# BrunoudA/MH-PPO

Hardware: AMD Instinct MI355X
Metric: env-steps/sec at 65536 envs × 4 agents, 1/2/4/8 MI355X + %HBM roofline (higher is better)
Workload: dtype f64 env / f32 nets; 1 GPU; config 3: 4cars nb_car=4 nb_ped=1 nb_lines=2, 65536 envs/GPU x 80 steps, full PPO iteration (rollout + returns + 10+10 epochs); envs_per_gpu=65536, agents=4, T=80, parallelism=dp1

## Files before the change

### include/mhppo.h

```cpp
#ifndef MHPPO_H
#define MHPPO_H
#include <stdint.h>

#ifdef __cplusplus
extern "C" {
#endif

#define MHPPO_OK 0
#define MHPPO_EINVAL -1
#define MHPPO_EHIP -2
#define MHPPO_ENOMEM -3
#define MHPPO_ENAN -4

#define MHPPO_COOP 0
#define MHPPO_4CARS 1
#define MHPPO_SCALABLE 2
#define MHPPO_NAIF 3
#define MHPPO_4CARS2 4
#define MHPPO_STOP 5
#define MHPPO_FIX_SCALABLE_LANES 1
#define MHPPO_GENERIC_STEP 2

typedef struct mhppo_env_cfg {
    int32_t variant;
// ... 111 lines not shown

int mhppo_libm_eval(int fn, uint64_t first, int64_t n, float *out, void *stream);

int mhppo_returns_scan(const double *rew, float *ret, int64_t B, int32_t T, double gamma, void *stream);
int mhppo_returns_scan_tm(const double *rew, float *ret, int64_t B, int32_t T, double gamma, void *stream);

typedef struct {
  float *obs, *act, *logp, *ret;
  double *rew;
} mhppo_bucket_dst;
int mhppo_bucket_scatter(const int64_t *pos, const int8_t *bucket, int64_t NS, int32_t T, const float *obs_tm,
                         const float *act_tm, const float *logp_tm, const float *ret_tm, const double *rew_tm,
                         const mhppo_bucket_dst *dst, void *stream);

int mhppo_bucket_scatter_sums(const int64_t *pos, const int8_t *bucket, int64_t NS, int32_t T, const float *obs_tm,
                              const float *act_tm, const float *logp_tm, const float *ret_tm, const double *rew_tm,
                              const mhppo_bucket_dst *dst, double *rew_sums, void *work, void *stream);

typedef struct {
  int64_t n_cross, n_wait, n_all, status;
  double counts[2];
  double rew_sums[3];
} mhppo_bucket_info;
int64_t mhppo_bucket_work_bytes(int64_t NS, int32_t T);
int mhppo_bucket_plan(int64_t N, int32_t S, int32_t P, int32_t dc, const int32_t *a_d, const int32_t *closest,
                      const uint8_t *exist, const int32_t *rec_of, const double *ep_min, const float *feat_d,
                      const float *logp_d, int32_t fix_bucket, const int32_t *status, int64_t *pos, int8_t *bucket,
                      float *c_obs, int32_t *c_act, float *c_logp, float *c_ret, mhppo_bucket_info *info,
                      void *work, void *stream);

int mhppo_adv_stats(const float *ret, const float *value, int64_t M, double *stats, void *stream);
int mhppo_adv_normalize(const float *ret, const float *value, int64_t M, const double *stats,
                        double m_global, float *adv, void *stream);

int mhppo_ppo_cont_fwd_bwd(const float *mu, const float *act, const float *logp_old,
                           const float *adv, int64_t M, double inv_m, float *dmu,
                           double *loss, void *stream);

int mhppo_ppo_choice_fwd_bwd(const float *probs, const float *logp_old, const float *adv,
                             int64_t M, const double *counts, double inv_m2, float *dprobs,
                             double *loss, void *stream);

#define MHPPO_TRAIN_EXACT_F32 0x100
int mhppo_mlp_train(int kind, int n_in, const float *packed, const float *X, int64_t M, const float *ret,
                    float *value, const float *act, const float *logp_old, const double *stats,
                    const double *counts, double m_global, float out_mean, float out_std, float *grad,
                    double *sums, void *stream);

int mhppo_mlp_train_pair(const float *packed_actor, const float *packed_critic, const float *X, int64_t M,
                         const float *ret, float *value, const float *act, const float *logp_old,
                         const double *stats, double m_global, float out_mean, float out_std,
                         float *grad_actor, double *sums_actor, float *grad_critic, double *sums_critic,
                         void *stream);

int mhppo_mse_fwd_bwd(const float *value, const float *ret, int64_t M, double inv_m, float *dv,
                      double *loss, void *stream);


int mhppo_mlp_forward(const mhppo_mlp *net, const float *X, int64_t M, float *out, void *stream);

#define MHPPO_DIAG_DSUM   0
#define MHPPO_DIAG_K3     1
#define MHPPO_DIAG_CLIP   2
#define MHPPO_DIAG_RATIO  3
#define MHPPO_DIAG_ENT    4
#define MHPPO_DIAG_E      5
#define MHPPO_DIAG_E2     6
#define MHPPO_DIAG_G      7
#define MHPPO_DIAG_G2     8
#define MHPPO_DIAG_V      9
#define MHPPO_DIAG_N     10
int64_t mhppo_ppo_diag_work_bytes(int64_t M);
int mhppo_ppo_diag(const mhppo_mlp *actor, const mhppo_mlp *critic, const float *X, int64_t M,
                   const void *act, const float *logp_old, const float *ret, double *sums,
                   void *work, void *stream);


int mhppo_gae_tm(const mhppo_mlp *critic0, const mhppo_mlp *critic1, const float *obs_tm,
                 const double *rew_tm, const int64_t *pos, const int8_t *bucket, int64_t B, int32_t T,
                 double gamma, double lambda, float *ret_tm, float *value_tm, void *stream);


#define MHPPO_EVS_ROWS       0
#define MHPPO_EVS_V0         1
#define MHPPO_EVS_V0_SQ      2
#define MHPPO_EVS_ABSA0      3
#define MHPPO_EVS_A0         4
#define MHPPO_EVS_A0_SQ      5
#define MHPPO_EVS_ABSVP0     6
#define MHPPO_EVS_ABSVP0_SQ  7
#define MHPPO_EVS_EPISODES   8
#define MHPPO_EVS_N_PED      9
#define MHPPO_EVS_PEDT      10
#define MHPPO_EVS_PEDT_SQ   11
#define MHPPO_EVS_WAIT      12
#define MHPPO_EVS_WAIT_SQ   13
#define MHPPO_EVS_N_CAR     14
#define MHPPO_EVS_CART      15
#define MHPPO_EVS_CART_SQ   16
#define MHPPO_EVS_FC        17
#define MHPPO_EVS_IC        18
#define MHPPO_EVS_N_YSPEED  19
#define MHPPO_EVS_YSPEED    20
#define MHPPO_EVS_YSPEED_SQ 21
#define MHPPO_EVS_N_YTIME   22
#define MHPPO_EVS_YTIME     23
// ... 72 lines not shown
```

### mh-ppo_amd/csrc/mlp_grad_reduce.h

```cpp
#pragma once
#include <hip/hip_runtime.h>

namespace {
constexpr int RG = 64;

template <class T>
__global__ void __launch_bounds__(256)
    k_grad_stage1(const T *gpart, const double *dpart, int nw, int np, double *tmp) {
  const int k = blockIdx.x * 256 + threadIdx.x;
  const int g = blockIdx.y, nd = np + 3, z = blockIdx.z;
  gpart += (size_t)z * nw * np;
  dpart += (size_t)z * nw * 3;
  tmp += (size_t)z * RG * nd;
  const int i0 = (int)((int64_t)g * nw / RG), i1 = (int)((int64_t)(g + 1) * nw / RG);
  double s = 0.0;
  if (k < np) {
#pragma unroll 16
    for (int i = i0; i < i1; i++) s += (double)gpart[(size_t)i * np + k];
  } else if (k < nd) {
    for (int i = i0; i < i1; i++) s += dpart[(size_t)i * 3 + (k - np)];
  } else {
    return;
  }
  tmp[(size_t)g * nd + k] = s;
}

constexpr int RD_COLS = 64, RD_GROUPS = 16;
__global__ void __launch_bounds__(RD_COLS * RD_GROUPS)
    k_grad_reduce_blocks(const double *gpart, const double *dpart, int nb, int np, float *grad, double *out3,
                         float *grad1, double *out3_1) {
  __shared__ double red[RD_GROUPS][RD_COLS];
  const int c = blockIdx.x * RD_COLS + (threadIdx.x & (RD_COLS - 1)), g = threadIdx.x / RD_COLS;
  const int nd = np + 3;
  if (blockIdx.y) {
    gpart += (size_t)nb * np;
    dpart += (size_t)nb * 3;
    grad = grad1;
    out3 = out3_1;
  }
  const int i0 = g * nb / RD_GROUPS, i1 = (g + 1) * nb / RD_GROUPS;
  double s = 0.0;
  if (c < np) {
#pragma unroll 16
    for (int i = i0; i < i1; i++) s += gpart[(size_t)i * np + c];
  } else if (c < nd) {
    for (int i = i0; i < i1; i++) s += dpart[(size_t)i * 3 + (c - np)];
  }
  red[g][threadIdx.x & (RD_COLS - 1)] = s;
  __syncthreads();
  if (g != 0 || c >= nd) return;
  double t = 0.0;
#pragma unroll
  for (int q = 0; q < RD_GROUPS; q++) t += red[q][threadIdx.x];
  if (c < np)
    grad[c] = (float)t;
  else if (out3)
    out3[c - np] += t;
}

__global__ void __launch_bounds__(256)
    k_grad_stage2(const double *tmp, int np, float *grad, double *out3, float *grad1, double *out3_1) {
  const int k = blockIdx.x * 256 + threadIdx.x, nd = np + 3;
  if (k >= nd) return;
  if (blockIdx.z) {
    tmp += (size_t)RG * nd;
    grad = grad1;
    out3 = out3_1;
  }
  double s = 0.0;
#pragma unroll 8
  for (int g = 0; g < RG; g++) s += tmp[(size_t)g * nd + k];
  if (k < np)
    grad[k] = (float)s;
  else if (out3)
    out3[k - np] += s;
}
}
```

### mh-ppo_amd/csrc/mlp_train.hip

```cpp
#include <hip/hip_runtime.h>
#include <stdint.h>

#include <algorithm>

#include "../../include/mhppo.h"
#include "common.h"
#include "mlp_tile.h"
#include "mlp_train_f32.h"
#include "mlp_x3_prims.h"
#include "mlp_x3.h"
#include "mlp_grad_reduce.h"

namespace {
struct Work {
  float *g = nullptr;
  double *d = nullptr;
  double *t = nullptr;
  int nw = 0;
  double *g64() const {
    static_assert(x3::WAVES * sizeof(float) >= sizeof(double), "a block's wave slots hold its float64 partial");
    return reinterpret_cast<double *>(g);
  }
};
constexpr int WORK_STREAMS = 4;
Work g_work[mhppo::MAX_DEVICES][WORK_STREAMS];
hipStream_t g_work_stream[mhppo::MAX_DEVICES][WORK_STREAMS];
int g_work_used[mhppo::MAX_DEVICES] = {0};
bool ensure_work(Work &wk, int slots) {
  if (wk.nw >= slots) return true;
  if (wk.g) (void)hipFree(wk.g);
  if (wk.d) (void)hipFree(wk.d);
  if (wk.t) (void)hipFree(wk.t);
  if (hipMalloc(&wk.g, sizeof(float) * (size_t)slots * NW_MAX) != hipSuccess ||
      hipMalloc(&wk.d, sizeof(double) * (size_t)slots * 3) != hipSuccess ||
      hipMalloc(&wk.t, sizeof(double) * (size_t)2 * RG * (NW_MAX + 3)) != hipSuccess) {
    wk = Work{};
    return false;
  }
  wk.nw = slots;
  return true;
}
Work *device_work(int dev, hipStream_t s) {
  int k = 0;
  while (k < g_work_used[dev] && g_work_stream[dev][k] != s) k++;
  if (k == g_work_used[dev]) {
    if (k == WORK_STREAMS) return nullptr;
    g_work_stream[dev][k] = s;
    g_work_used[dev] = k + 1;
  }
  return &g_work[dev][k];
}

struct Launch {
  Work *wk;
  int blocks, nw;
};
enum XAlign { X_ANY, X_16B_BEFORE_LOOKUP, X_16B_AFTER_LOOKUP };
int prepare_launch(hipStream_t s, int64_t M, const float *X, XAlign xa, int waves, int nets, Launch &L) {
  if (M > ((int64_t)1 << 40)) return set_error(MHPPO_EINVAL, "M too large");
  const bool misaligned = ((uintptr_t)X & 15) != 0;
  if (xa == X_16B_BEFORE_LOOKUP && misaligned)
    return set_error(MHPPO_EINVAL, "X must be 16-byte aligned (LDS-DMA rows)");
  int dev = 0;
  CHECK_HIP(hipGetDevice(&dev));
  if (dev < 0 || dev >= mhppo::MAX_DEVICES) return set_error(MHPPO_EINVAL, "device %d >= %d", dev, mhppo::MAX_DEVICES);
  L.wk = device_work(dev, s);
  if (!L.wk) return set_error(MHPPO_EINVAL, "train passes on more than %d streams of one device", WORK_STREAMS);
  if (xa == X_16B_AFTER_LOOKUP && misaligned)
    return set_error(MHPPO_EINVAL, "X must be 16-byte aligned (LDS-DMA rows)");
  const int64_t tiles = (M + 31) / 32;
  L.blocks = (int)std::max<int64_t>(1, std::min<int64_t>(mhppo::device_cus(dev), (tiles + waves - 1) / waves));
  L.nw = L.blocks * waves;
  if (!ensure_work(*L.wk, nets * L.nw)) return set_error(MHPPO_ENOMEM, "mlp_train partials");
  return MHPPO_OK;
}

using X3Kernel = decltype(&k_mlp_train_x3<K_CRITIC, x3::G13S>);
struct X3Launch {
  X3Kernel kernel;
  int lds_bytes;
};
template <int KIND, class G>
constexpr X3Launch x3_of() { return {k_mlp_train_x3<KIND, G>, G::LDS_BYTES}; }
X3Launch x3_kernel(int kind, int n_in) {
  using namespace x3;
  const bool critic = kind == K_CRITIC;
  if (n_in == NIN_CONT && kind != K_CHOICE) return critic ? x3_of<K_CRITIC, G13S>() : x3_of<K_CONT, G13S>();
  if (n_in <= 15) return critic ? x3_of<K_CRITIC, GV16>() : x3_of<K_CHOICE, GC16>();
  if (n_in <= 31) return critic ? x3_of<K_CRITIC, GV32>() : x3_of<K_CHOICE, GC32>();
  if (n_in == 54) return critic ? x3_of<K_CRITIC, GV54>() : x3_of<K_CHOICE, GC54>();
  return critic ? x3_of<K_CRITIC, GV64>() : x3_of<K_CHOICE, GC64>();
}
using F32Launch = decltype(&launch<K_CRITIC, 7, true>);
F32Launch f32_launcher(int kind, int n_in) {
  if (n_in == NIN_CONT && kind != K_CHOICE)
    return kind == K_CRITIC ? launch<K_CRITIC, 7, true> : launch<K_CONT, 7, true>;
  static constexpr F32Launch CRITIC[6] = {launch<K_CRITIC, 8, false>,  launch<K_CRITIC, 12, false>,
                                          launch<K_CRITIC, 16, false>, launch<K_CRITIC, 24, false>,
                                          launch<K_CRITIC, 28, false>, launch<K_CRITIC, 32, false>};
  static constexpr F32Launch CHOICE[6] = {launch<K_CHOICE, 8, false>,  launch<K_CHOICE, 12, false>,
                                          launch<K_CHOICE, 16, false>, launch<K_CHOICE, 24, false>,
                                          launch<K_CHOICE, 28, false>, launch<K_CHOICE, 32, false>};
  const int w = n_in <= 16 ? 0 : (n_in <= 24 ? 1 : (n_in <= 32 ? 2 : (n_in <= 48 ? 3 : (n_in <= 56 ? 4 : 5))));
  return (kind == K_CRITIC ? CRITIC : CHOICE)[w];
}
}

#ifdef MHPPO_TIMING
extern "C" int mhppo_debug_timing_train(unsigned long long *out16) {
  CHECK_HIP(hipDeviceSynchronize());
  CHECK_HIP(hipMemcpyFromSymbol(out16, HIP_SYMBOL(g_timing), sizeof(unsigned long long) * 16));
  unsigned long long z[16] = {0};
  CHECK_HIP(hipMemcpyToSymbol(HIP_SYMBOL(g_timing), z, sizeof(z)));
  return MHPPO_OK;
}
#endif

extern "C" int mhppo_mlp_train(int kind, int n_in, const float *packed, const float *X, int64_t M, const float *ret,
                               float *value, const float *act, const float *logp_old, const double *stats,
                               const double *counts, double m_global, float out_mean, float out_std, float *grad,
                               double *sums, void *stream) {
  const bool exact = (kind & MHPPO_TRAIN_EXACT_F32) != 0;
  kind &= ~MHPPO_TRAIN_EXACT_F32;
  if (!grad || M < 0 || kind < K_CRITIC || kind > K_CHOICE || n_in < 1 || n_in > NIN_MAX)
    return set_error(MHPPO_EINVAL, "bad argument (kind 0..2 [| MHPPO_TRAIN_EXACT_F32], 1 <= n_in <= %d)", NIN_MAX);
  hipStream_t s = (hipStream_t)stream;
  const int np = n_params(n_in, kind == K_CHOICE ? 2 : 1);
  if (M == 0) {
    CHECK_HIP(hipMemsetAsync(grad, 0, sizeof(float) * np, s));
    return MHPPO_OK;
  }
  if (!packed || !X || !ret || !value) return set_error(MHPPO_EINVAL, "null packed/X/ret/value");
  if (kind == K_CONT && (n_in != NIN_CONT || !act || !logp_old || !stats))
    return set_error(MHPPO_EINVAL, "continuous actor pass needs n_in 13 and act/logp_old/stats");
  if (kind == K_CHOICE && (!logp_old || !stats || (!counts && !act)))
    return set_error(MHPPO_EINVAL, "choice actor pass needs logp_old/stats and counts (or act for per-row mode)");
  const bool pf = n_in == NIN_CONT && kind != K_CHOICE;
  const bool split = !exact && (pf || n_in <= x3::NIN_X3C);
  const int waves = split ? x3::WAVES : (pf ? 8 : 4);
  Launch L;
  const int rc = prepare_launch(s, M, X, pf ? X_16B_BEFORE_LOOKUP : (split ? X_16B_AFTER_LOOKUP : X_ANY), waves, 1, L);
  if (rc != MHPPO_OK) return rc;
  Work &wk = *L.wk;
  const dim3 grid((unsigned)L.blocks);
  if (split) {
    const X3Launch k = x3_kernel(kind, n_in);
    hipLaunchKernelGGL(k.kernel, grid, dim3(64 * x3::WAVES), k.lds_bytes, s, packed, X, n_in, M, ret, value, act,
                       logp_old, stats, counts, m_global, out_mean, out_std, wk.g64(), wk.d);
    hipLaunchKernelGGL(k_grad_reduce_blocks, dim3((np + 3 + RD_COLS - 1) / RD_COLS), dim3(RD_COLS * RD_GROUPS), 0, s,
                       wk.g64(), wk.d, L.blocks, np, grad, sums, nullptr, nullptr);
  } else {
    f32_launcher(kind, n_in)(grid, s, packed, X, n_in, M, ret, value, act, logp_old, stats, counts, m_global, out_mean,
                             out_std, wk.g, wk.d);
    hipLaunchKernelGGL(k_grad_stage1<float>, dim3((np + 3 + 255) / 256, RG), dim3(256), 0, s, wk.g, wk.d, L.nw, np,
                       wk.t);
    hipLaunchKernelGGL(k_grad_stage2, dim3((np + 3 + 255) / 256), dim3(256), 0, s, wk.t, np, grad, sums, nullptr,
                       nullptr);
  }
  CHECK_HIP(hipGetLastError());
  return MHPPO_OK;
}

extern "C" int mhppo_mlp_train_pair(const float *packed_actor, const float *packed_critic, const float *X, int64_t M,
                                    const float *ret, float *value, const float *act, const float *logp_old,
                                    const double *stats, double m_global, float out_mean, float out_std,
                                    float *grad_actor, double *sums_actor, float *grad_critic, double *sums_critic,
                                    void *stream) {
  if (!grad_actor || !grad_critic || M < 0) return set_error(MHPPO_EINVAL, "bad argument");
  hipStream_t s = (hipStream_t)stream;
  const int np = n_params(NIN_CONT, 1);
  if (M == 0) {
    CHECK_HIP(hipMemsetAsync(grad_actor, 0, sizeof(float) * np, s));
    CHECK_HIP(hipMemsetAsync(grad_critic, 0, sizeof(float) * np, s));
    return MHPPO_OK;
  }
  if (!packed_actor || !packed_critic || !X || !ret || !value || !act || !logp_old || !stats)
    return set_error(MHPPO_EINVAL, "null pointer");
  Launch L;
  const int rc = prepare_launch(s, M, X, X_16B_BEFORE_LOOKUP, x3::WAVES, 2, L);
  if (rc != MHPPO_OK) return rc;
  Work &wk = *L.wk;
  hipLaunchKernelGGL(k_mlp_train_x3_pair, dim3((unsigned)L.blocks), dim3(64 * x3::WAVES), x3::G13::LDS_BYTES_PAIR, s,
                     packed_actor, packed_critic, X, M, ret, value, act, logp_old, stats, m_global, out_mean, out_std,
                     wk.g64(), wk.d);
  hipLaunchKernelGGL(k_grad_reduce_blocks, dim3((np + 3 + RD_COLS - 1) / RD_COLS, 2), dim3(RD_COLS * RD_GROUPS), 0, s,
                     wk.g64(), wk.d, L.blocks, np, grad_actor, sums_actor, grad_critic, sums_critic);
  CHECK_HIP(hipGetLastError());
  return MHPPO_OK;
}
```

### mh-ppo_amd/mhppo/_lib.py

```python
import ctypes
import os

HERE = os.path.dirname(os.path.abspath(__file__))
LIB_PATH = os.environ.get("MHPPO_LIB") or os.path.join(HERE, "lib", "libmhppo.so")

P = ctypes.c_void_p
I32 = ctypes.c_int32
I64 = ctypes.c_int64
U64 = ctypes.c_uint64
F64 = ctypes.c_double


class EnvCfg(ctypes.Structure):
    _fields_ = [
        ("variant", I32), ("n_envs", I32), ("nb_car", I32), ("nb_ped", I32), ("nb_lines", I32),
        ("max_episode", I32), ("sin_model", I32), ("flags", I32), ("dt", F64),
        ("car_b", F64 * 4), ("ped_b", F64 * 8), ("cross_b", F64 * 2), ("seed_base", U64),
        ("env_id_offset", U64),
    ]


class Mlp(ctypes.Structure):
    _fields_ = [("packed", P), ("n_in", I32), ("n_out", I32), ("kind", I32), ("reserved", I32),
                ("mean", ctypes.c_float), ("std", ctypes.c_float)]


class BucketDst(ctypes.Structure):
    _fields_ = [("obs", P), ("act", P), ("logp", P), ("ret", P), ("rew", P)]


class RolloutBufs(ctypes.Structure):
    _fields_ = [("feat_d", P), ("probs_d", P), ("logp_d", P), ("a_d", P), ("closest", P),
                ("feat_c", P), ("out_c", P), ("obs", P), ("obs_c", P), ("act", P), ("logp", P),
                ("rew", P), ("ep_min", P), ("exist", P), ("rows", P), ("T", I32),
                ("flags", I32), ("status", P), ("parts", I32), ("reserved", I32), ("rec_of", P)]


class EvalBufs(ctypes.Structure):
    _fields_ = [("obs", P), ("a_d", P), ("trig", P), ("ep_min", P), ("obs_hist", P), ("acts", P), ("rews_c", P),
                ("rews_d", P), ("waiting", P), ("saved", P), ("T", I32), ("reserved", I32)]


class PolicyNoise(ctypes.Structure):
    _fields_ = [("tape", P), ("forced", P), ("key", U64), ("first_env", U64), ("t", I64)]


class AdamSeg(ctypes.Structure):
    _fields_ = [("param", P), ("grad", P), ("exp_avg", P), ("exp_avg_sq", P), ("step", P), ("n", I64)]


ADAM_MAX_NETS, ADAM_MAX_SEGS = 8, 8


class AdamNet(ctypes.Structure):
    _fields_ = [("seg", AdamSeg * ADAM_MAX_SEGS), ("n_seg", I32), ("reserved", I32), ("t", I64), ("alpha", F64),
                ("bias2", F64), ("beta1", F64), ("beta2", F64), ("eps", F64)]


_SIGS = {
    "mhppo_env_create": (I32, [ctypes.POINTER(EnvCfg), I32, ctypes.POINTER(P)]),
    "mhppo_env_destroy": (None, [P]),
    "mhppo_env_obs_dim": (I32, [P]),
    "mhppo_env_slots": (I32, [P]),
    "mhppo_env_reward_slots": (I32, [P]),
    "mhppo_env_state_dim": (I32, [P]),
    "mhppo_env_reset": (I32, [P, P, P]),
    "mhppo_env_choix_test": (I32, [P, P, P]),
    "mhppo_env_state_bytes": (I64, [P]),
    "mhppo_env_export": (I32, [P, P, P]),
    "mhppo_env_import": (I32, [P, P, P]),
    "mhppo_env_step": (I32, [P, P, P, P, P, P, P]),
    "mhppo_env_get_state": (I32, [P, P, P]),
    "mhppo_env_get_rng": (I32, [P, P, P, P]),
    "mhppo_env_events": (I32, [P, P, P]),
    "mhppo_choice_dim": (I32, [P]),
    "mhppo_rollout_begin": (I32, [P, ctypes.POINTER(Mlp), P, P, ctypes.POINTER(RolloutBufs), P]),
    "mhppo_rollout_step": (I32, [P, ctypes.POINTER(Mlp), ctypes.POINTER(Mlp), P, I32,
                                 ctypes.POINTER(RolloutBufs), P]),
    "mhppo_rollout_policy": (I32, [P, ctypes.POINTER(Mlp), ctypes.POINTER(Mlp), ctypes.POINTER(RolloutBufs), P]),
    "mhppo_rollout_sample_env": (I32, [P, P, I32, ctypes.POINTER(RolloutBufs), P]),
    "mhppo_rollout_policy_part": (I32, [P, ctypes.POINTER(Mlp), ctypes.POINTER(Mlp), ctypes.POINTER(RolloutBufs), I32,
                                        P]),
    "mhppo_rollout_sample_env_part": (I32, [P, P, I32, ctypes.POINTER(RolloutBufs), I32, P]),
    "mhppo_kernel_timing_begin": (I32, [I32]),
    "mhppo_kernel_timing_end": (I32, [ctypes.POINTER(ctypes.c_double), ctypes.POINTER(I32)]),
    "mhppo_kernel_timing_end_each": (I32, [P, I32, ctypes.POINTER(I32)]),
    "mhppo_eval_step": (I32, [P, ctypes.POINTER(Mlp), ctypes.POINTER(Mlp), ctypes.POINTER(Mlp), I32,
                              ctypes.POINTER(EvalBufs), P]),
    "mhppo_rollout_check": (I32, [ctypes.POINTER(RolloutBufs), P]),
    "mhppo_philox_normal": (I32, [U64, U64, P, I64, P]),
    "mhppo_philox_uniform": (I32, [U64, U64, P, I64, P]),
    "mhppo_philox_normal_2d": (I32, [U64, U64, U64, P, I64, I64, P]),
    "mhppo_libm_eval": (I32, [I32, U64, I64, P, P]),
    "mhppo_returns_scan": (I32, [P, P, I64, I32, F64, P]),
    "mhppo_returns_scan_tm": (I32, [P, P, I64, I32, F64, P]),
    "mhppo_bucket_scatter": (I32, [P, P, I64, I32] + [P] * 7),
    "mhppo_bucket_scatter_sums": (I32, [P, P, I64, I32] + [P] * 9),
    "mhppo_bucket_work_bytes": (I64, [I64, I32]),
    "mhppo_bucket_plan": (I32, [I64, I32, I32, I32] + [P] * 7 + [I32] + [P] * 10),
    "mhppo_adv_stats": (I32, [P, P, I64, P, P]),
    "mhppo_adv_normalize": (I32, [P, P, I64, P, F64, P, P]),
    "mhppo_ppo_cont_fwd_bwd": (I32, [P, P, P, P, I64, F64, P, P, P]),
    "mhppo_ppo_choice_fwd_bwd": (I32, [P, P, P, I64, P, F64, P, P, P]),
    "mhppo_mse_fwd_bwd": (I32, [P, P, I64, F64, P, P, P]),
    "mhppo_mlp_train": (I32, [I32, I32, P, P, I64, P, P, P, P, P, P, F64, ctypes.c_float, ctypes.c_float, P, P, P]),
    "mhppo_mlp_train_pair": (I32, [P, P, P, I64, P, P, P, P, P, F64, ctypes.c_float, ctypes.c_float, P, P, P, P, P]),
    "mhppo_mlp_forward": (I32, [ctypes.POINTER(Mlp), P, I64, P, P]),
    "mhppo_ppo_diag_work_bytes": (I64, [I64]),
    "mhppo_ppo_diag": (I32, [ctypes.POINTER(Mlp), ctypes.POINTER(Mlp), P, I64, P, P, P, P, P, P]),
    "mhppo_gae_tm": (I32, [ctypes.POINTER(Mlp), ctypes.POINTER(Mlp), P, P, P, P, I64, I32, F64, F64, P, P, P]),
    "mhppo_eval_stats_bytes": (I64, [P]),
    "mhppo_eval_stats_begin": (I32, [P, P, P]),
    "mhppo_eval_stats_row": (I32, [P, P, I32, I32, P, P]),
    "mhppo_eval_stats_fold": (I32, [P, P, P, P]),
    "mhppo_adam_clip": (I32, [P, I32, F64, P, P]),
    "mhppo_batch_shuffle": (I32, [I32, I64, P, P, P, P, U64, I32, P, P, P, P, P, P]),
    "mhppo_policy_dims": (I32, [ctypes.POINTER(EnvCfg), P]),
    "mhppo_policy_decide": (I32, [ctypes.POINTER(EnvCfg), ctypes.POINTER(Mlp), P, I64, P, P, P]),
    "mhppo_policy_act": (I32, [ctypes.POINTER(EnvCfg), ctypes.POINTER(Mlp), ctypes.POINTER(Mlp), P, P, I64, P, P]),
    "mhppo_policy_sample_decide": (I32, [ctypes.POINTER(EnvCfg), ctypes.POINTER(Mlp), P, I64,
                                         ctypes.POINTER(PolicyNoise)] + [P] * 8),
    "mhppo_policy_sample_act": (I32, [ctypes.POINTER(EnvCfg), ctypes.POINTER(Mlp), ctypes.POINTER(Mlp), P, P, P, I64,
                                      ctypes.POINTER(PolicyNoise)] + [P] * 6),
    "mhppo_last_error": (ctypes.c_char_p, []),
    "mhppo_version": (ctypes.c_char_p, []),
}

_lib = None


class MhppoError(RuntimeError):
    pass


class MhppoNaNError(MhppoError, ValueError):
    """MHPPO_ENAN: a NaN policy output was sampled (the reference raises ValueError there)."""

ENAN = -4
MHPPO_ROLLOUT_VALU_POLICY = 1
MHPPO_ROLLOUT_VALU_UNSORTED = 2


def lib():
    global _lib
    if _lib is None:
        if not os.path.exists(LIB_PATH):
            raise MhppoError(f"{LIB_PATH} is missing: build it with `python -c 'import __graft_entry__ as g; g.build()'`")
        L = ctypes.CDLL(LIB_PATH)
        for name, (res, args) in _SIGS.items():
            fn = getattr(L, name)
            fn.restype = res
            fn.argtypes = args
        _lib = L
    return _lib


def declared_symbols():
    return list(_SIGS)

# ... 52 lines not shown
```

### mh-ppo_amd/mhppo/ppo.py

```python
import contextlib
import ctypes
import math
import os

import torch
import torch.distributed as dist

from . import _lib
from .adam import adam_clip_steps, adam_clip_sumsq, adam_clip_torch, adam_steps, clip_forget, fold_1024_4


_FORCE_COLLECTIVES = False


def set_force_collectives(flag=True):
    global _FORCE_COLLECTIVES
    _FORCE_COLLECTIVES = bool(flag)


def _dp():
    if not (dist.is_available() and dist.is_initialized()):
        return False
    return _FORCE_COLLECTIVES or dist.get_world_size() > 1

# ... 273 lines not shown
        self.per_row = per_row
        self.exact = bool(exact)


PIPELINE_PAIRS = {"0": False, "1": True}.get(os.environ.get("MHPPO_PIPELINE_PAIRS", ""), None)
PAIR_MAX_ROWS = 2_000_000


def _use_pair(h):
    if h.kind != "c" or h.exact:
        return False
    return PIPELINE_PAIRS if PIPELINE_PAIRS is not None else h.m <= PAIR_MAX_ROWS


class _HeadPlan:

    def __init__(self, h):
        cont = h.kind == "c"
        self.akind = KIND_CONT if cont else KIND_CHOICE
        _check_net(KIND_CRITIC, h.critic)
        _check_net(self.akind, h.actor)
        self.obs, self.ret = _obs_rows(h.obs), h.ret.float().contiguous()
        self.M = self.obs.shape[0]
        self.lp = h.logp.float().contiguous()
        self.act = h.act.float().contiguous() if (cont or h.per_row) else None
        self.counts = None if (cont or h.per_row) else h.counts
        self.V = torch.empty(self.M, dtype=torch.float32, device=self.obs.device)
        self.n_in = h.actor.n_in
        self.keep = (h.actor.flat(), h.critic.flat())
        self.wa, self.wc = self.keep[0].data_ptr(), self.keep[1].data_ptr()
        self.ga, self.gc = h.actor.grad_flat().data_ptr(), h.critic.grad_flat().data_ptr()
        self.mean, self.std = float(h.actor.mean), float(h.actor.std)
        self.flags = TRAIN_EXACT_F32 if h.exact else 0
        self.pair = _use_pair(h) and self.M > 0
        self.x, self.r, self.v, self.l = (t.data_ptr() for t in (self.obs, self.ret, self.V, self.lp))
        self.a, self.cn = _addr(self.act), _addr(self.counts)


def _critic_pass(p, h, sums, st):
    _launch_train(KIND_CRITIC, p.flags, p.n_in, p.wc, p.x, p.M, p.r, p.v, None, None, None, None, h.m, 0.0, 1.0, p.gc,
                  sums.data_ptr(), st)


def _actor_pass(p, h, stats, sums, st):
    _launch_train(p.akind, p.flags, p.n_in, p.wa, p.x, p.M, p.r, p.v, p.a, p.l, stats.data_ptr(), p.cn, h.m, p.mean,
                  p.std, p.ga, sums.data_ptr(), st)


def _pair_pass(p, h, stats, sums_a, sums_c, st):
    _launch_pair(p.wa, p.wc, p.x, p.M, p.r, p.v, p.a, p.l, stats.data_ptr(), h.m, p.mean, p.std, p.ga,
                 sums_a.data_ptr(), p.gc, sums_c.data_ptr(), st)


def _on_device(dev):
    return torch.cuda.device(dev) if dev.type == "cuda" else contextlib.nullcontext()


def _reduce_and_step(nets, opts, bucket, max_grad_norm, norms_out):
    if bucket is not None:
        bucket.allreduce(nets)
    else:
        _allreduce_net_grads(*nets)
    if max_grad_norm is None:
        adam_steps(opts)
    elif opts:
        adam_steps(opts, max_grad_norm, norms_out)


def train_epoch(heads, bucket=None, max_grad_norm=None, norms_out=None):
    H = len(heads)
    dev = heads[0].obs.device
    with _on_device(dev):
        st = torch.cuda.current_stream(dev).cuda_stream if dev.type == "cuda" else None
        sums = torch.zeros(2 * H, 3, dtype=torch.float64, device=dev)
        plans = [_HeadPlan(h) for h in heads]
        for i, (p, h) in enumerate(zip(plans, heads)):
            _critic_pass(p, h, sums[i], st)
        stats = sums[:H, 1:3].reshape(-1).contiguous()
        _allreduce_(stats)
        for i, (p, h) in enumerate(zip(plans, heads)):
            _actor_pass(p, h, stats[2 * i:2 * i + 2], sums[H + i], st)
        _reduce_and_step([n for h in heads for n in (h.actor, h.critic)],
                         [o for h in heads for o in (h.opt_actor, h.opt_critic)], bucket, max_grad_norm, norms_out)
    return [(sums[H + i, 0:1], sums[i, 0:1]) for i in range(H)]


TRAIN_STREAMS = max(1, int(os.environ.get("MHPPO_TRAIN_STREAMS", "1")))
_SIDE_STREAMS = {}


def _side_streams(dev, n):
    if dev.type != "cuda" or n <= 0:
        return []
    key = (dev.index if dev.index is not None else torch.cuda.current_device(), n)
    if key not in _SIDE_STREAMS:
        _SIDE_STREAMS[key] = [torch.cuda.Stream(device=dev) for _ in range(n)]
    return _SIDE_STREAMS[key]


def train_epochs(heads, n_epochs, bucket=None, max_grad_norm=None):
    H = len(heads)
    dev = heads[0].obs.device
    with _on_device(dev):
        norms = None
        if max_grad_norm is not None:
            norms = torch.full((n_epochs, 2 * H), math.nan, dtype=torch.float64, device=dev)
        all_sums = torch.zeros(n_epochs + 1, 2 * H, 3, dtype=torch.float64, device=dev)
        dp = _dp()
        plans = [_HeadPlan(h) for h in heads]
        main = torch.cuda.current_stream(dev) if dev.type == "cuda" else None
        side = _side_streams(dev, min(TRAIN_STREAMS, H) - 1)
        streams = [main] + side
        handles = [None if s is None else s.cuda_stream for s in streams]
        same_stream = contextlib.nullcontext()
        stats = None
        out = [[None, None] for _ in range(H)]
        for k in range(n_epochs + 1):
            sums = all_sums[k]
            crit = k < n_epochs
            trained = []
            if side:
                fork = torch.cuda.Event()
                fork.record(main)
                for sd in side:
                    sd.wait_event(fork)
            for i, h in enumerate(heads):
                p = plans[i]
                sc, sa = sums[i], sums[H + i]
                j = i % len(streams)
                st = handles[j]
                with (torch.cuda.stream(streams[j]) if side else same_stream):
                    stp = None
                    if k > 0:
                        stp = stats[2 * i:2 * i + 2] if dp else all_sums[k - 1, i, 1:3]
                    if k > 0 and crit and p.pair:
                        _pair_pass(p, h, stp, sa, sc, st)
                    else:
                        if k > 0:
                            _actor_pass(p, h, stp, sa, st)
                        if crit:
                            _critic_pass(p, h, sc, st)
                if k > 0:
                    trained.append(h.actor)
                    out[i][0] = sums[H + i, 0:1]
                if crit:
                    trained.append(h.critic)
                    out[i][1] = sums[i, 0:1]
            for sd in side:
                main.wait_stream(sd)
            if crit and dp:
                stats = sums[:H, 1:3].reshape(-1).contiguous()
                _allreduce_(stats)
            opts = ([h.opt_actor for h in heads] if k > 0 else []) + ([h.opt_critic for h in heads] if crit else [])
            nout = None
            if norms is not None:
                off = (k - 1) * 2 * H + H if k > 0 else 0
                nout = norms.view(-1)[off:off + len(opts)]
            _reduce_and_step(trained, opts, bucket, max_grad_norm, nout)
    if norms is not None:
        return [tuple(o) for o in out], norms
    return [tuple(o) for o in out]



class _SliceHead:

    def __init__(self, h, m):
        self.actor, self.critic, self.kind, self.m = h.actor, h.critic, h.kind, float(m)


class _SlicePlan:

    def __init__(self, p, b0, b1, counts):
        for k in ("akind", "n_in", "wa", "wc", "ga", "gc", "mean", "std", "flags", "keep"):
            setattr(self, k, getattr(p, k))
        self.pair = False
        self.M = b1 - b0
        self.obs, self.ret, self.V, self.lp = p.obs[b0:b1], p.ret[b0:b1], p.V[b0:b1], p.lp[b0:b1]
        self.act = None if p.act is None else p.act[b0:b1]
        self.counts = counts
        self.x, self.r, self.v, self.l = p.x + 4 * self.n_in * b0, p.r + 4 * b0, p.v + 4 * b0, p.l + 4 * b0
        self.a = None if p.a is None else p.a + 4 * b0
        self.cn = _addr(counts)


def train_minibatches(heads, n_epochs, K, key_fn, bucket=None, max_grad_norm=None, slice_m=None):
    from . import shuffle
    H, K = len(heads), int(K)
    if K < 1:
        raise ValueError(f"K must be >= 1, not {K}")
    dev = heads[0].obs.device
    with _on_device(dev):
        st = torch.cuda.current_stream(dev).cuda_stream if dev.type == "cuda" else None
        dp = _dp()
        n_choice = sum(1 for h in heads if h.kind != "c" and not h.per_row)
        counts_all = torch.zeros(max(1, n_choice), K, 2, dtype=torch.float64, device=dev)
        srcs, dsts, cnts, plans = [], [], [], []
        for h in heads:
            fl = h.kind == "c" or h.per_row
            act = h.act.float().contiguous() if fl else h.act.to(torch.int32).contiguous()
            src = (h.obs.float().contiguous(), act, h.logp.float().contiguous(), h.ret.float().contiguous())
            dst = tuple(torch.empty_like(t) for t in src)
# ... 63 lines not shown
```

Baseline: 79.63 million env-steps/s.

## Batch all per-epoch train passes into one native call with shared gradient reduce

Adds mhppo_train_step, which takes a table of actor, critic and pair passes for every head. It launches them in one native call across at most two streams, joins the streams, and then runs a single table-driven gradient-reduce kernel over all nets. This replaces many per-head Python/ctypes calls, per-pass reduce launches and torch side-stream event plumbing. The goal is lower host dispatch and launch overhead in the PPO epochs, at the cost of a serialized reduce after the join and a limit of two streams.

```diff
diff --git a/include/mhppo.h b/include/mhppo.h
--- a/include/mhppo.h
+++ b/include/mhppo.h
@@ -187,6 +187,31 @@
                          const double *stats, double m_global, float out_mean, float out_std,
                          float *grad_actor, double *sums_actor, float *grad_critic, double *sums_critic,
                          void *stream);
+
+#define MHPPO_TRAIN_STEP_MAX_PASSES 16
+typedef struct mhppo_train_pass {
+  int32_t pair;
+  int32_t head;
+  int32_t kind;
+  int32_t n_in;
+  const float *packed;
+  const float *packed_critic;
+  const float *X;
+  int64_t M;
+  const float *ret;
+  float *value;
+  const float *act;
+  const float *logp_old;
+  const double *stats;
+  const double *counts;
+  double m_global;
+  float out_mean, out_std;
+  float *grad;
+  double *sums;
+  float *grad_critic;
+  double *sums_critic;
+} mhppo_train_pass;
+int mhppo_train_step(const mhppo_train_pass *passes, int n_passes, int streams, void *stream);
 
 int mhppo_mse_fwd_bwd(const float *value, const float *ret, int64_t M, double inv_m, float *dv,
                       double *loss, void *stream);
diff --git a/mh-ppo_amd/csrc/mlp_grad_reduce.h b/mh-ppo_amd/csrc/mlp_grad_reduce.h
--- a/mh-ppo_amd/csrc/mlp_grad_reduce.h
+++ b/mh-ppo_amd/csrc/mlp_grad_reduce.h
@@ -1,5 +1,7 @@
 #pragma once
 #include <hip/hip_runtime.h>
+
+#include "../../include/mhppo.h"
 
 namespace {
 constexpr int RG = 64;
@@ -26,18 +28,22 @@
 }
 
 constexpr int RD_COLS = 64, RD_GROUPS = 16;
-__global__ void __launch_bounds__(RD_COLS * RD_GROUPS)
-    k_grad_reduce_blocks(const double *gpart, const double *dpart, int nb, int np, float *grad, double *out3,
-                         float *grad1, double *out3_1) {
+struct ReduceNet {
+  const double *gpart, *dpart;
+  float *grad;
+  double *out3;
+  int nb, np;
+};
+constexpr int RD_MAX_NETS = 2 * MHPPO_TRAIN_STEP_MAX_PASSES;
+struct ReduceTable {
+  ReduceNet net[RD_MAX_NETS];
+};
+__global__ void __launch_bounds__(RD_COLS * RD_GROUPS) k_grad_reduce_blocks(const ReduceTable tab) {
   __shared__ double red[RD_GROUPS][RD_COLS];
   const int c = blockIdx.x * RD_COLS + (threadIdx.x & (RD_COLS - 1)), g = threadIdx.x / RD_COLS;
-  const int nd = np + 3;
-  if (blockIdx.y) {
-    gpart += (size_t)nb * np;
-    dpart += (size_t)nb * 3;
-    grad = grad1;
-    out3 = out3_1;
-  }
+  const ReduceNet &n = tab.net[blockIdx.y];
+  const double *gpart = n.gpart, *dpart = n.dpart;
+  const int nb = n.nb, np = n.np, nd = np + 3;
   const int i0 = g * nb / RD_GROUPS, i1 = (g + 1) * nb / RD_GROUPS;
   double s = 0.0;
   if (c < np) {
@@ -53,9 +59,15 @@
 #pragma unroll
   for (int q = 0; q < RD_GROUPS; q++) t += red[q][threadIdx.x];
   if (c < np)
-    grad[c] = (float)t;
-  else if (out3)
-    out3[c - np] += t;
+    n.grad[c] = (float)t;
+  else if (n.out3)
+    n.out3[c - np] += t;
+}
+inline void launch_reduce_blocks(const ReduceTable &tab, int nets, hipStream_t s) {
+  int np = 0;
+  for (int i = 0; i < nets; i++) np = tab.net[i].np > np ? tab.net[i].np : np;
+  hipLaunchKernelGGL(k_grad_reduce_blocks, dim3((np + 3 + RD_COLS - 1) / RD_COLS, nets), dim3(RD_COLS * RD_GROUPS), 0,
+                     s, tab);
 }
 
 __global__ void __launch_bounds__(256)
diff --git a/mh-ppo_amd/csrc/mlp_train.hip b/mh-ppo_amd/csrc/mlp_train.hip
--- a/mh-ppo_amd/csrc/mlp_train.hip
+++ b/mh-ppo_amd/csrc/mlp_train.hip
@@ -55,6 +55,10 @@
   Work *wk;
   int blocks, nw;
 };
+int grid_blocks(int dev, int64_t M, int waves) {
+  const int64_t tiles = (M + 31) / 32;
+  return (int)std::max<int64_t>(1, std::min<int64_t>(mhppo::device_cus(dev), (tiles + waves - 1) / waves));
+}
 enum XAlign { X_ANY, X_16B_BEFORE_LOOKUP, X_16B_AFTER_LOOKUP };
 int prepare_launch(hipStream_t s, int64_t M, const float *X, XAlign xa, int waves, int nets, Launch &L) {
   if (M > ((int64_t)1 << 40)) return set_error(MHPPO_EINVAL, "M too large");
@@ -68,8 +72,7 @@
   if (!L.wk) return set_error(MHPPO_EINVAL, "train passes on more than %d streams of one device", WORK_STREAMS);
   if (xa == X_16B_AFTER_LOOKUP && misaligned)
     return set_error(MHPPO_EINVAL, "X must be 16-byte aligned (LDS-DMA rows)");
-  const int64_t tiles = (M + 31) / 32;
-  L.blocks = (int)std::max<int64_t>(1, std::min<int64_t>(mhppo::device_cus(dev), (tiles + waves - 1) / waves));
+  L.blocks = grid_blocks(dev, M, waves);
   L.nw = L.blocks * waves;
   if (!ensure_work(*L.wk, nets * L.nw)) return set_error(MHPPO_ENOMEM, "mlp_train partials");
   return MHPPO_OK;
@@ -104,6 +107,84 @@
   const int w = n_in <= 16 ? 0 : (n_in <= 24 ? 1 : (n_in <= 32 ? 2 : (n_in <= 48 ? 3 : (n_in <= 56 ? 4 : 5))));
   return (kind == K_CRITIC ? CRITIC : CHOICE)[w];
 }
+
+int check_single(int kind, int n_in, const float *packed, const float *X, int64_t M, const float *ret,
+                 const float *value, const float *act, const float *logp_old, const double *stats,
+                 const double *counts, const float *grad) {
+  if (!grad || M < 0 || kind < K_CRITIC || kind > K_CHOICE || n_in < 1 || n_in > NIN_MAX)
+    return set_error(MHPPO_EINVAL, "bad argument (kind 0..2 [| MHPPO_TRAIN_EXACT_F32], 1 <= n_in <= %d)", NIN_MAX);
+  if (M == 0) return MHPPO_OK;
+  if (!packed || !X || !ret || !value) return set_error(MHPPO_EINVAL, "null packed/X/ret/value");
+  if (kind == K_CONT && (n_in != NIN_CONT || !act || !logp_old || !stats))
+    return set_error(MHPPO_EINVAL, "continuous actor pass needs n_in 13 and act/logp_old/stats");
+  if (kind == K_CHOICE && (!logp_old || !stats || (!counts && !act)))
+    return set_error(MHPPO_EINVAL, "choice actor pass needs logp_old/stats and counts (or act for per-row mode)");
+  return MHPPO_OK;
+}
+int check_pair(const float *packed_actor, const float *packed_critic, const float *X, int64_t M, const float *ret,
+               const float *value, const float *act, const float *logp_old, const double *stats,
+               const float *grad_actor, const float *grad_critic) {
+  if (!grad_actor || !grad_critic || M < 0) return set_error(MHPPO_EINVAL, "bad argument");
+  if (M == 0) return MHPPO_OK;
+  if (!packed_actor || !packed_critic || !X || !ret || !value || !act || !logp_old || !stats)
+    return set_error(MHPPO_EINVAL, "null pointer");
+  return MHPPO_OK;
+}
+struct SingleShape {
+  bool pf, split;
+  int waves, np;
+};
+SingleShape single_shape(int kind, int n_in, bool exact) {
+  SingleShape sh;
+  sh.pf = n_in == NIN_CONT && kind != K_CHOICE;
+  sh.split = !exact && (sh.pf || n_in <= x3::NIN_X3C);
+  sh.waves = sh.split ? x3::WAVES : (sh.pf ? 8 : 4);
+  sh.np = n_params(n_in, kind == K_CHOICE ? 2 : 1);
+  return sh;
+}
+
+struct Step {
+  hipStream_t side = nullptr;
+  hipEvent_t fork = nullptr, join = nullptr;
+  double *g = nullptr, *d = nullptr;
+  size_t ng = 0, nd = 0;
+};
+Step g_step[mhppo::MAX_DEVICES];
+int ensure_step_lane(Step &st) {
+  if (st.side) return MHPPO_OK;
+  hipStream_t side = nullptr;
+  hipEvent_t fork = nullptr, join = nullptr;
+  if (hipStreamCreateWithFlags(&side, hipStreamNonBlocking) != hipSuccess ||
+      hipEventCreateWithFlags(&fork, hipEventDisableTiming) != hipSuccess ||
+      hipEventCreateWithFlags(&join, hipEventDisableTiming) != hipSuccess) {
+    if (join) (void)hipEventDestroy(join);
+    if (fork) (void)hipEventDestroy(fork);
+    if (side) (void)hipStreamDestroy(side);
+    return set_error(MHPPO_EHIP, "mhppo_train_step: side stream / events");
+  }
+  st.side = side, st.fork = fork, st.join = join;
+  return MHPPO_OK;
+}
+bool ensure_step_work(Step &st, size_t ng, size_t nd) {
+  if (st.ng < ng) {
+    if (st.g) (void)hipFree(st.g);
+    st.g = nullptr, st.ng = 0;
+    if (hipMalloc(&st.g, sizeof(double) * ng) != hipSuccess) return false;
+    st.ng = ng;
+  }
+  if (st.nd < nd) {
+    if (st.d) (void)hipFree(st.d);
+    st.d = nullptr, st.nd = 0;
+    if (hipMalloc(&st.d, sizeof(double) * nd) != hipSuccess) return false;
+    st.nd = nd;
+  }
+  return true;
+}
+int check_rows(int64_t M, const float *X, bool need_16b) {
+  if (M > ((int64_t)1 << 40)) return set_error(MHPPO_EINVAL, "M too large");
+  if (need_16b && ((uintptr_t)X & 15) != 0) return set_error(MHPPO_EINVAL, "X must be 16-byte aligned (LDS-DMA rows)");
+  return MHPPO_OK;
+}
 }
 
 #ifdef MHPPO_TIMING
@@ -116,42 +197,53 @@
 }
 #endif
 
+namespace {
+void launch_x3(int kind, int n_in, int blocks, hipStream_t s, const float *packed, const float *X, int64_t M,
+               const float *ret, float *value, const float *act, const float *logp_old, const double *stats,
+               const double *counts, double m_global, float out_mean, float out_std, double *gpart, double *dpart) {
+  const X3Launch k = x3_kernel(kind, n_in);
+  hipLaunchKernelGGL(k.kernel, dim3((unsigned)blocks), dim3(64 * x3::WAVES), k.lds_bytes, s, packed, X, n_in, M, ret,
+                     value, act, logp_old, stats, counts, m_global, out_mean, out_std, gpart, dpart);
+}
+void launch_x3_pair(int blocks, hipStream_t s, const float *packed_actor, const float *packed_critic, const float *X,
+                    int64_t M, const float *ret, float *value, const float *act, const float *logp_old,
+                    const double *stats, double m_global, float out_mean, float out_std, double *gpart,
+                    double *dpart) {
+  hipLaunchKernelGGL(k_mlp_train_x3_pair, dim3((unsigned)blocks), dim3(64 * x3::WAVES), x3::G13::LDS_BYTES_PAIR, s,
+                     packed_actor, packed_critic, X, M, ret, value, act, logp_old, stats, m_global, out_mean, out_std,
+                     gpart, dpart);
+}
+}
+
 extern "C" int mhppo_mlp_train(int kind, int n_in, const float *packed, const float *X, int64_t M, const float *ret,
                                float *value, const float *act, const float *logp_old, const double *stats,
                                const double *counts, double m_global, float out_mean, float out_std, float *grad,
                                double *sums, void *stream) {
   const bool exact = (kind & MHPPO_TRAIN_EXACT_F32) != 0;
   kind &= ~MHPPO_TRAIN_EXACT_F32;
-  if (!grad || M < 0 || kind < K_CRITIC || kind > K_CHOICE || n_in < 1 || n_in > NIN_MAX)
-    return set_error(MHPPO_EINVAL, "bad argument (kind 0..2 [| MHPPO_TRAIN_EXACT_F32], 1 <= n_in <= %d)", NIN_MAX);
+  const int rc0 = check_single(kind, n_in, packed, X, M, ret, value, act, logp_old, stats, counts, grad);
+  if (rc0 != MHPPO_OK) return rc0;
   hipStream_t s = (hipStream_t)stream;
-  const int np = n_params(n_in, kind == K_CHOICE ? 2 : 1);
+  const SingleShape sh = single_shape(kind, n_in, exact);
+  const int np = sh.np;
   if (M == 0) {
     CHECK_HIP(hipMemsetAsync(grad, 0, sizeof(float) * np, s));
     return MHPPO_OK;
   }
-  if (!packed || !X || !ret || !value) return set_error(MHPPO_EINVAL, "null packed/X/ret/value");
-  if (kind == K_CONT && (n_in != NIN_CONT || !act || !logp_old || !stats))
-    return set_error(MHPPO_EINVAL, "continuous actor pass needs n_in 13 and act/logp_old/stats");
-  if (kind == K_CHOICE && (!logp_old || !stats || (!counts && !act)))
-    return set_error(MHPPO_EINVAL, "choice actor pass needs logp_old/stats and counts (or act for per-row mode)");
-  const bool pf = n_in == NIN_CONT && kind != K_CHOICE;
-  const bool split = !exact && (pf || n_in <= x3::NIN_X3C);
-  const int waves = split ? x3::WAVES : (pf ? 8 : 4);
   Launch L;
-  const int rc = prepare_launch(s, M, X, pf ? X_16B_BEFORE_LOOKUP : (split ? X_16B_AFTER_LOOKUP : X_ANY), waves, 1, L);
+  const int rc = prepare_launch(s, M, X, sh.pf ? X_16B_BEFORE_LOOKUP : (sh.split ? X_16B_AFTER_LOOKUP : X_ANY),
+                                sh.waves, 1, L);
   if (rc != MHPPO_OK) return rc;
   Work &wk = *L.wk;
-  const dim3 grid((unsigned)L.blocks);
-  if (split) {
-    const X3Launch k = x3_kernel(kind, n_in);
-    hipLaunchKernelGGL(k.kernel, grid, dim3(64 * x3::WAVES), k.lds_bytes, s, packed, X, n_in, M, ret, value, act,
-                       logp_old, stats, counts, m_global, out_mean, out_std, wk.g64(), wk.d);
-    hipLaunchKernelGGL(k_grad_reduce_blocks, dim3((np + 3 + RD_COLS - 1) / RD_COLS), dim3(RD_COLS * RD_GROUPS), 0, s,
-                       wk.g64(), wk.d, L.blocks, np, grad, sums, nullptr, nullptr);
+  if (sh.split) {
+    launch_x3(kind, n_in, L.blocks, s, packed, X, M, ret, value, act, logp_old, stats, counts, m_global, out_mean,
+              out_std, wk.g64(), wk.d);
+    ReduceTable tab = {};
+    tab.net[0] = {wk.g64(), wk.d, grad, sums, L.blocks, np};
+    launch_reduce_blocks(tab, 1, s);
   } else {
-    f32_launcher(kind, n_in)(grid, s, packed, X, n_in, M, ret, value, act, logp_old, stats, counts, m_global, out_mean,
-                             out_std, wk.g, wk.d);
+    f32_launcher(kind, n_in)(dim3((unsigned)L.blocks), s, packed, X, n_in, M, ret, value, act, logp_old, stats, counts,
+                             m_global, out_mean, out_std, wk.g, wk.d);
     hipLaunchKernelGGL(k_grad_stage1<float>, dim3((np + 3 + 255) / 256, RG), dim3(256), 0, s, wk.g, wk.d, L.nw, np,
                        wk.t);
     hipLaunchKernelGGL(k_grad_stage2, dim3((np + 3 + 255) / 256), dim3(256), 0, s, wk.t, np, grad, sums, nullptr,
@@ -166,7 +258,9 @@
                                     const double *stats, double m_global, float out_mean, float out_std,
                                     float *grad_actor, double *sums_actor, float *grad_critic, double *sums_critic,
                                     void *stream) {
-  if (!grad_actor || !grad_critic || M < 0) return set_error(MHPPO_EINVAL, "bad argument");
+  const int rc0 = check_pair(packed_actor, packed_critic, X, M, ret, value, act, logp_old, stats, grad_actor,
+                             grad_critic);
+  if (rc0 != MHPPO_OK) return rc0;
   hipStream_t s = (hipStream_t)stream;
   const int np = n_params(NIN_CONT, 1);
   if (M == 0) {
@@ -174,17 +268,109 @@
     CHECK_HIP(hipMemsetAsync(grad_critic, 0, sizeof(float) * np, s));
     return MHPPO_OK;
   }
-  if (!packed_actor || !packed_critic || !X || !ret || !value || !act || !logp_old || !stats)
-    return set_error(MHPPO_EINVAL, "null pointer");
   Launch L;
   const int rc = prepare_launch(s, M, X, X_16B_BEFORE_LOOKUP, x3::WAVES, 2, L);
   if (rc != MHPPO_OK) return rc;
   Work &wk = *L.wk;
-  hipLaunchKernelGGL(k_mlp_train_x3_pair, dim3((unsigned)L.blocks), dim3(64 * x3::WAVES), x3::G13::LDS_BYTES_PAIR, s,
-                     packed_actor, packed_critic, X, M, ret, value, act, logp_old, stats, m_global, out_mean, out_std,
-                     wk.g64(), wk.d);
-  hipLaunchKernelGGL(k_grad_reduce_blocks, dim3((np + 3 + RD_COLS - 1) / RD_COLS, 2), dim3(RD_COLS * RD_GROUPS), 0, s,
-                     wk.g64(), wk.d, L.blocks, np, grad_actor, sums_actor, grad_critic, sums_critic);
+  launch_x3_pair(L.blocks, s, packed_actor, packed_critic, X, M, ret, value, act, logp_old, stats, m_global, out_mean,
+                 out_std, wk.g64(), wk.d);
+  ReduceTable tab = {};
+  tab.net[0] = {wk.g64(), wk.d, grad_actor, sums_actor, L.blocks, np};
+  tab.net[1] = {wk.g64() + (size_t)L.blocks * np, wk.d + (size_t)L.blocks * 3, grad_critic, sums_critic, L.blocks, np};
+  launch_reduce_blocks(tab, 2, s);
   CHECK_HIP(hipGetLastError());
   return MHPPO_OK;
 }
+
+extern "C" int mhppo_train_step(const mhppo_train_pass *passes, int n_passes, int streams, void *stream) {
+  if (n_passes < 0 || n_passes > MHPPO_TRAIN_STEP_MAX_PASSES || (n_passes > 0 && !passes) || streams < 1 || streams > 2)
+    return set_error(MHPPO_EINVAL, "mhppo_train_step: 0 <= n_passes <= %d pass records, 1 or 2 streams",
+                     MHPPO_TRAIN_STEP_MAX_PASSES);
+  for (int i = 0; i < n_passes; i++) {
+    const mhppo_train_pass &p = passes[i];
+    if (p.head < 0) return set_error(MHPPO_EINVAL, "mhppo_train_step: pass %d has a negative head", i);
+    int rc;
+    bool need_16b = true;
+    if (p.pair) {
+      rc = check_pair(p.packed, p.packed_critic, p.X, p.M, p.ret, p.value, p.act, p.logp_old, p.stats, p.grad,
+                      p.grad_critic);
+    } else {
+      const int kind = p.kind & ~MHPPO_TRAIN_EXACT_F32;
+      rc = check_single(kind, p.n_in, p.packed, p.X, p.M, p.ret, p.value, p.act, p.logp_old, p.stats, p.counts, p.grad);
+      if (rc == MHPPO_OK) {
+        const SingleShape sh = single_shape(kind, p.n_in, (p.kind & MHPPO_TRAIN_EXACT_F32) != 0);
+        need_16b = sh.pf || sh.split;
+      }
+    }
+    if (rc == MHPPO_OK && p.M > 0) rc = check_rows(p.M, p.X, need_16b);
+    if (rc != MHPPO_OK) return rc;
+  }
+  if (n_passes == 0) return MHPPO_OK;
+  hipStream_t s = (hipStream_t)stream;
+  int dev = 0;
+  CHECK_HIP(hipGetDevice(&dev));
+  if (dev < 0 || dev >= mhppo::MAX_DEVICES) return set_error(MHPPO_EINVAL, "device %d >= %d", dev, mhppo::MAX_DEVICES);
+  Step &st = g_step[dev];
+  struct Slot {
+    size_t g, d;
+    int blocks, np;
+  } slot[MHPPO_TRAIN_STEP_MAX_PASSES];
+  size_t ng = 0, nd = 0;
+  bool side = false;
+  for (int i = 0; i < n_passes; i++) {
+    const mhppo_train_pass &p = passes[i];
+    side = side || p.head % streams != 0;
+    slot[i] = {ng, nd, 0, n_params(NIN_CONT, 1)};
+    if (p.M == 0) continue;
+    if (!p.pair) {
+      const int kind = p.kind & ~MHPPO_TRAIN_EXACT_F32;
+      const SingleShape sh = single_shape(kind, p.n_in, (p.kind & MHPPO_TRAIN_EXACT_F32) != 0);
+      if (!sh.split) continue;
+      slot[i].np = sh.np;
+    }
+    slot[i].blocks = grid_blocks(dev, p.M, x3::WAVES);
+    const size_t nets = p.pair ? 2 : 1;
+    ng += nets * slot[i].blocks * slot[i].np;
+    nd += nets * slot[i].blocks * 3;
+  }
+  if (!ensure_step_work(st, ng, nd)) return set_error(MHPPO_ENOMEM, "mhppo_train_step partials");
+  if (side) {
+    const int rc = ensure_step_lane(st);
+    if (rc != MHPPO_OK) return rc;
+    CHECK_HIP(hipEventRecord(st.fork, s));
+    CHECK_HIP(hipStreamWaitEvent(st.side, st.fork, 0));
+  }
+  ReduceTable tab = {};
+  int nets = 0, rc = MHPPO_OK;
+  for (int i = 0; i < n_passes && rc == MHPPO_OK; i++) {
+    const mhppo_train_pass &p = passes[i];
+    hipStream_t lane = p.head % streams ? st.side : s;
+    const Slot &sl = slot[i];
+    double *g = st.g + sl.g, *d = st.d + sl.d;
+    if (sl.blocks == 0) {
+      rc = p.pair ? mhppo_mlp_train_pair(p.packed, p.packed_critic, p.X, p.M, p.ret, p.value, p.act, p.logp_old, p.stats,
+                                         p.m_global, p.out_mean, p.out_std, p.grad, p.sums, p.grad_critic,
+                                         p.sums_critic, lane)
+                  : mhppo_mlp_train(p.kind, p.n_in, p.packed, p.X, p.M, p.ret, p.value, p.act, p.logp_old, p.stats,
+                                    p.counts, p.m_global, p.out_mean, p.out_std, p.grad, p.sums, lane);
+    } else if (p.pair) {
+      launch_x3_pair(sl.blocks, lane, p.packed, p.packed_critic, p.X, p.M, p.ret, p.value, p.act, p.logp_old, p.stats,
+                     p.m_global, p.out_mean, p.out_std, g, d);
+      tab.net[nets++] = {g, d, p.grad, p.sums, sl.blocks, sl.np};
+      tab.net[nets++] = {g + (size_t)sl.blocks * sl.np, d + (size_t)sl.blocks * 3, p.grad_critic, p.sums_critic,
+                         sl.blocks, sl.np};
+    } else {
+      launch_x3(p.kind, p.n_in, sl.blocks, lane, p.packed, p.X, p.M, p.ret, p.value, p.act, p.logp_old, p.stats,
+                p.counts, p.m_global, p.out_mean, p.out_std, g, d);
+      tab.net[nets++] = {g, d, p.grad, p.sums, sl.blocks, sl.np};
+    }
+  }
+  if (side) {
+    CHECK_HIP(hipEventRecord(st.join, st.side));
+    CHECK_HIP(hipStreamWaitEvent(s, st.join, 0));
+  }
+  if (rc != MHPPO_OK) return rc;
+  if (nets > 0) launch_reduce_blocks(tab, nets, s);
+  CHECK_HIP(hipGetLastError());
+  return MHPPO_OK;
+}
diff --git a/mh-ppo_amd/mhppo/_lib.py b/mh-ppo_amd/mhppo/_lib.py
--- a/mh-ppo_amd/mhppo/_lib.py
+++ b/mh-ppo_amd/mhppo/_lib.py
@@ -48,6 +48,15 @@
 class AdamSeg(ctypes.Structure):
     _fields_ = [("param", P), ("grad", P), ("exp_avg", P), ("exp_avg_sq", P), ("step", P), ("n", I64)]
 
+
+class TrainPass(ctypes.Structure):
+    _fields_ = [("pair", I32), ("head", I32), ("kind", I32), ("n_in", I32), ("packed", P), ("packed_critic", P),
+                ("X", P), ("M", I64), ("ret", P), ("value", P), ("act", P), ("logp_old", P), ("stats", P),
+                ("counts", P), ("m_global", F64), ("out_mean", ctypes.c_float), ("out_std", ctypes.c_float),
+                ("grad", P), ("sums", P), ("grad_critic", P), ("sums_critic", P)]
+
+
+TRAIN_STEP_MAX_PASSES = 16
 
 ADAM_MAX_NETS, ADAM_MAX_SEGS = 8, 8
 
@@ -105,6 +114,7 @@
     "mhppo_mse_fwd_bwd": (I32, [P, P, I64, F64, P, P, P]),
     "mhppo_mlp_train": (I32, [I32, I32, P, P, I64, P, P, P, P, P, P, F64, ctypes.c_float, ctypes.c_float, P, P, P]),
     "mhppo_mlp_train_pair": (I32, [P, P, P, I64, P, P, P, P, P, F64, ctypes.c_float, ctypes.c_float, P, P, P, P, P]),
+    "mhppo_train_step": (I32, [P, I32, I32, P]),
     "mhppo_mlp_forward": (I32, [ctypes.POINTER(Mlp), P, I64, P, P]),
     "mhppo_ppo_diag_work_bytes": (I64, [I64]),
     "mhppo_ppo_diag": (I32, [ctypes.POINTER(Mlp), ctypes.POINTER(Mlp), P, I64, P, P, P, P, P, P]),
diff --git a/mh-ppo_amd/mhppo/ppo.py b/mh-ppo_amd/mhppo/ppo.py
--- a/mh-ppo_amd/mhppo/ppo.py
+++ b/mh-ppo_amd/mhppo/ppo.py
@@ -349,6 +349,44 @@
                  sums_a.data_ptr(), p.gc, sums_c.data_ptr(), st)
 
 
+_PASS_HELPERS = (_critic_pass, _actor_pass, _pair_pass)
+
+
+class _StepRecords:
+
+    def __init__(self, plans, heads, actors, critics):
+        rows = []
+        for i, (p, h) in enumerate(zip(plans, heads)):
+            if actors and critics and p.pair:
+                rows.append((i, "pair"))
+            else:
+                rows += [(i, "actor")] * actors + [(i, "critic")] * critics
+        self.rows = rows
+        self.arr = (_lib.TrainPass * max(1, len(rows)))()
+        for r, (i, role) in zip(self.arr, rows):
+            p, h = plans[i], heads[i]
+            r.head, r.X, r.M, r.ret, r.value, r.m_global = i, p.x, p.M, p.r, p.v, h.m
+            if role == "critic":
+                r.kind, r.n_in, r.packed, r.grad = KIND_CRITIC | p.flags, p.n_in, p.wc, p.gc
+                r.out_mean, r.out_std = 0.0, 1.0
+                continue
+            r.packed, r.grad, r.act, r.logp_old, r.out_mean, r.out_std = p.wa, p.ga, p.a, p.l, p.mean, p.std
+            if role == "pair":
+                r.pair, r.packed_critic, r.grad_critic = 1, p.wc, p.gc
+            else:
+                r.kind, r.n_in, r.counts = p.akind | p.flags, p.n_in, p.cn
+        self.addr = ctypes.addressof(self.arr)
+
+    def point(self, H, sums, stats, stats_stride):
+        for r, (i, role) in zip(self.arr, self.rows):
+            if role == "critic":
+                r.sums = sums + 24 * i
+                continue
+            r.stats, r.sums = stats + stats_stride * i, sums + 24 * (H + i)
+            if role == "pair":
+                r.sums_critic = sums + 24 * i
+
+
 def _on_device(dev):
     return torch.cuda.device(dev) if dev.type == "cuda" else contextlib.nullcontext()
 
@@ -406,7 +444,14 @@
         dp = _dp()
         plans = [_HeadPlan(h) for h in heads]
         main = torch.cuda.current_stream(dev) if dev.type == "cuda" else None
-        side = _side_streams(dev, min(TRAIN_STREAMS, H) - 1)
+        step_call = (dev.type == "cuda" and TRAIN_EVENTS is None and 2 * H <= _lib.TRAIN_STEP_MAX_PASSES
+                     and (_critic_pass, _actor_pass, _pair_pass) == _PASS_HELPERS)
+        if step_call:
+            step_fn, main_handle = _lib.lib().mhppo_train_step, main.cuda_stream
+            step_streams = min(TRAIN_STREAMS, H, 2)
+            shapes = {}
+            sums0 = all_sums.data_ptr()
+        side = [] if step_call else _side_streams(dev, min(TRAIN_STREAMS, H) - 1)
         streams = [main] + side
         handles = [None if s is None else s.cuda_stream for s in streams]
         same_stream = contextlib.nullcontext()
@@ -415,13 +460,23 @@
         for k in range(n_epochs + 1):
             sums = all_sums[k]
             crit = k < n_epochs
-            trained = []
+            if step_call:
+                recs = shapes.get((k > 0, crit))
+                if recs is None:
+                    recs = shapes[(k > 0, crit)] = _StepRecords(plans, heads, k > 0, crit)
+                if k == 0:
+                    recs.point(H, sums0, 0, 0)
+                elif dp:
+                    recs.point(H, sums0 + 48 * H * k, stats.data_ptr(), 16)
+                else:
+                    recs.point(H, sums0 + 48 * H * k, sums0 + 48 * H * (k - 1) + 8, 24)
+                _lib.check(step_fn(recs.addr, len(recs.rows), step_streams, main_handle))
             if side:
                 fork = torch.cuda.Event()
                 fork.record(main)
                 for sd in side:
                     sd.wait_event(fork)
-            for i, h in enumerate(heads):
+            for i, h in enumerate(() if step_call else heads):
                 p = plans[i]
                 sc, sa = sums[i], sums[H + i]
                 j = i % len(streams)
@@ -437,14 +492,16 @@
                             _actor_pass(p, h, stp, sa, st)
                         if crit:
                             _critic_pass(p, h, sc, st)
+            for sd in side:
+                main.wait_stream(sd)
+            trained = []
+            for i, h in enumerate(heads):
                 if k > 0:
                     trained.append(h.actor)
                     out[i][0] = sums[H + i, 0:1]
                 if crit:
                     trained.append(h.critic)
                     out[i][1] = sums[i, 0:1]
-            for sd in side:
-                main.wait_stream(sd)
             if crit and dp:
                 stats = sums[:H, 1:3].reshape(-1).contiguous()
                 _allreduce_(stats)
```

Result: no change. 79.44 million env-steps/s (-0.2%).
